# gashon/transformer-lm

Measured on AMD Instinct MI355X. Metric: BPE train input MB/s (32k vocab), train_bpe(path) end to end, higher is better.
Workload: dtype int64

## Files before the change

transformer-lm_amd/csrc/api.hip:

```cpp
#include <dlfcn.h>
#include <hip/hip_version.h>

#include <cerrno>
#include <cstdio>
#include <cstdlib>
#include <cstring>
#include <fstream>
#include <memory>
#include <mutex>
#include <string_view>
#include <unordered_map>
#include <unordered_set>
#include <string>
#include <vector>

#include "count.h"
#include "drive.h"
#include "internal.h"

namespace bpe {

namespace {
thread_local std::string g_err;
thread_local int g_errno = 0;
// ... 134 lines not shown
}

}

extern "C" {

int bpe_abi_version(void) { return BPE355_ABI_VERSION; }

int bpe_runtime_info(int* compiled_hip_version, int* runtime_hip_version, char* runtime_path, size_t cap) {
    if (compiled_hip_version) *compiled_hip_version = HIP_VERSION;
    int rv = 0;
    const hipError_t e = hipRuntimeGetVersion(&rv);
    if (runtime_hip_version) *runtime_hip_version = e == hipSuccess ? rv : 0;
    if (runtime_path && cap) {
        runtime_path[0] = '\0';
        Dl_info di{};
        if (dladdr(reinterpret_cast<void*>(&hipRuntimeGetVersion), &di) && di.dli_fname)
            std::snprintf(runtime_path, cap, "%s", di.dli_fname);
    }
    return e == hipSuccess ? BPE_OK : BPE_E_HIP;
}
const char* bpe_last_error(void) { return bpe::g_err.c_str(); }
int bpe_last_errno(void) { return bpe::g_errno; }
void bpe_set_timing(int enable) { bpe::g_timing = enable != 0; }

int bpe_release_device_memory(int device, size_t* freed_bytes) {
    return bpe::guarded([&] {
        if (freed_bytes) *freed_bytes = 0;
        int n = 0;
        if (hipGetDeviceCount(&n) != hipSuccess) n = 0;
        BPE_REQUIRE(device < n, BPE_E_ARG, "device " + std::to_string(device) + " is not visible");
        size_t b = bpe::corpus_release(device);
        b += bpe::scratch_release(device);
        if (freed_bytes) *freed_bytes = b;
    });
}

int bpe_device_count(void) {
    int n = 0;
    if (hipGetDeviceCount(&n) != hipSuccess) return 0;
    int k = 0;
    for (int i = 0; i < n; ++i) {
        hipDeviceProp_t p;
        if (hipGetDeviceProperties(&p, i) == hipSuccess && std::strncmp(p.gcnArchName, "gfx950", 6) == 0) ++k;
    }
    return k;
}

int bpe_train_device(const uint8_t* d_data, size_t n, int vocab_size, const char* const* specials,
                     int n_specials, bpe_comm* comm, void* hip_stream, bpe_result** out) {
    if (n && !d_data) return bpe::guarded([] { throw bpe::Error{BPE_E_ARG, "data is NULL"}; });
    return train_common(d_data, n, vocab_size, specials, n_specials, comm, hip_stream, out);
}

int bpe_train_buffer(const uint8_t* data, size_t n, int vocab_size, const char* const* specials,
                     int n_specials, bpe_comm* comm, bpe_result** out) {
    return bpe::guarded([&] {
        BPE_REQUIRE(out, BPE_E_ARG, "out is NULL");
        *out = nullptr;
        BPE_REQUIRE(!n || data, BPE_E_ARG, "data is NULL");
        bpe::DeviceGuard::require();
        auto sp = bpe::to_specials(specials, n_specials);
        const bpe::Source src = bpe::Source::memory(data, n);
        bpe::TrainOutput to;
        if (comm) bpe::train_source_comm(src, false, vocab_size, sp, comm->impl.get(), to);
        else bpe::train_source(src, vocab_size, sp, 1, to);
// ... 206 lines not shown
```

transformer-lm_amd/csrc/bpe_common.h:

```cpp
#pragma once

#include <hip/hip_runtime.h>

#include <cstddef>
#include <cstdint>
#include <string>

#include "../../include/bpe355.h"

namespace bpe {

void set_error(int code, const std::string& msg, int sys_errno = 0);
struct Error {
    int code;
    std::string msg;
    int sys_errno = 0;
};

#define BPE_HIP(expr)                                                                     \
    do {                                                                                  \
        hipError_t e_ = (expr);                                                           \
        if (e_ != hipSuccess)                                                             \
            throw ::bpe::Error{BPE_E_HIP, std::string(#expr) + ": " + hipGetErrorString(e_) + \
                                              " (" __FILE__ ":" + std::to_string(__LINE__) + ")"}; \
    } while (0)

#define BPE_REQUIRE(cond, code, msg)                          \
    do {                                                      \
        if (!(cond)) throw ::bpe::Error{(code), (msg)};       \
    } while (0)

template <class T>
struct DevBuf {
    T* p = nullptr;
    size_t n = 0;
    DevBuf() = default;
    explicit DevBuf(size_t count) { alloc(count); }
    DevBuf(const DevBuf&) = delete;
    DevBuf& operator=(const DevBuf&) = delete;
    DevBuf(DevBuf&& o) noexcept : p(o.p), n(o.n) { o.p = nullptr; o.n = 0; }
    DevBuf& operator=(DevBuf&& o) noexcept {
        if (this != &o) { release(); p = o.p; n = o.n; o.p = nullptr; o.n = 0; }
        return *this;
    }
    ~DevBuf() { release(); }
    void alloc(size_t count) {
        release();
        if (!count) return;
        const hipError_t e = hipMalloc(&p, count * sizeof(T));
        if (e == hipErrorOutOfMemory) {
            (void)hipGetLastError();
            p = nullptr;
            throw ::bpe::Error{BPE_E_NOMEM, "device allocation of " + std::to_string(count * sizeof(T)) +
                                                " bytes failed (out of memory)"};
        }
        BPE_HIP(e);
        n = count;
    }
    void reserve(size_t count) {
        if (count > n || !p) alloc(count);
    }
    void release() {
        if (p) (void)hipFree(p);
        p = nullptr;
        n = 0;
    }
    size_t bytes() const { return n * sizeof(T); }
};

enum : int { CLS_OTHER = 0, CLS_LETTER = 1, CLS_NUMBER = 2, CLS_SPACE = 3 };

__host__ __device__ inline uint64_t mix64(uint64_t z) {
    z ^= z >> 30; z *= 0xBF58476D1CE4E5B9ULL;
    z ^= z >> 27; z *= 0x94D049BB133111EBULL;
    return z ^ (z >> 31);
}

__device__ __forceinline__ unsigned wave_append(bool pred, unsigned* counter) {
    const unsigned long long m = __ballot(pred);
    if (!m) return ~0u;
    const int leader = __ffsll((long long)m) - 1;
    const unsigned lane = threadIdx.x & 63;
    unsigned base = 0;
    if ((int)lane == leader) base = atomicAdd(counter, (unsigned)__popcll(m));
    base = __shfl(base, leader);
    const unsigned below = __builtin_amdgcn_mbcnt_hi((unsigned)(m >> 32),
                                                     __builtin_amdgcn_mbcnt_lo((unsigned)m, 0u));
    return pred ? base + below : ~0u;
}

template <class T>
__device__ __forceinline__ T wave_sum(T v) {
    for (int o = 32; o > 0; o >>= 1) v += __shfl_xor(v, o);
    return v;
}

template <class T>
__device__ __forceinline__ T wave_max(T v) {
// ... 21 lines not shown
```

transformer-lm_amd/csrc/count.hip:

```cpp
#include <hip/hip_ext.h>

#include <algorithm>
#include <cstdlib>
#include <mutex>
#include <vector>

#include "count.h"
#include "pretok.h"
#include "prims.h"
#include "stage.h"
#include "stage2.h"
#include "tokstart.h"

#ifndef BPE355_COUNT_EARLY_PREFETCH
#define BPE355_COUNT_EARLY_PREFETCH 1
#endif

namespace bpe {

namespace {

constexpr int kCache2 = 512;
constexpr int kEpoch2 = 4;
constexpr unsigned kKeep2 = 2;
// ... 736 lines not shown
            } else {
                ++i;
            }
    }
    if (drop.empty()) return bytes;
    int cur = 0;
    BPE_HIP(hipGetDevice(&cur));
    for (auto& x : drop) {
        (void)hipSetDevice(x->dev);
        x.reset();
    }
    BPE_HIP(hipSetDevice(cur));
    return bytes;
}

void scratch_give(std::unique_ptr<Arrays3> x) {
    if (!x) return;
    std::lock_guard<std::mutex> g(scratch().m);
    scratch().free_.push_back(std::move(x));
}

RecPoolOwner::~RecPoolOwner() {
    scratch_give(std::move(rec));
    scratch_give(std::move(B));
}

void RecPoolOwner::init(size_t n_bytes, unsigned grid, hipStream_t s) {
    size_t want = std::max<size_t>(n_bytes / 10, (size_t)grid * kPageRecs);
    if (const char* e = std::getenv("BPE355_REC_POOL")) want = (size_t)std::atof(e);
    int dev = 0;
    BPE_HIP(hipGetDevice(&dev));
    size_t free_b = 0, total_b = 0;
    BPE_HIP(hipMemGetInfo(&free_b, &total_b));
    const size_t avail = free_b + scratch_cached_bytes(dev);
    const size_t reserve = std::max<size_t>(total_b / 16, n_bytes / 2);
    size_t fit = avail > reserve ? (avail - reserve) / (6 * sizeof(uint64_t) + 1) : 0;
    if (const char* e = std::getenv("BPE355_REC_POOL_FIT")) fit = (size_t)std::atof(e);
    if (fit < want) {
        if (fit < (size_t)grid * kPageRecs / 4)
            throw Error{BPE_E_NOMEM, "record pool: " + std::to_string(avail) + " bytes of device memory free"};
        want = fit;
    }
    max_pages = (unsigned)std::max<size_t>(1, std::min<size_t>((want + kPageRecs - 1) / kPageRecs, 1u << 30));
    const size_t cap = (size_t)max_pages * kPageRecs;
    if (std::getenv("BPE355_REC_POOL_FAIL"))
        throw Error{BPE_E_NOMEM, "record pool allocation failed (BPE355_REC_POOL_FAIL)"};
    rec = scratch_take(cap);
    page_used.alloc(max_pages);
    page_ch.alloc((size_t)max_pages * kCoarse);
    n_pages.alloc(1);
    wg_page.alloc(grid);
    wg_used.alloc(grid);
    wg_ch.alloc((size_t)grid * kCoarse);
    BPE_HIP(hipMemsetAsync(wg_ch.p, 0, 4ull * grid * kCoarse, s));
    held.alloc(max_pages);
    done.alloc(max_pages);
    lw_per_wg = (unsigned)std::min<size_t>(1u << 24, std::max<size_t>(1024, n_bytes / 1024 / grid + 1));
    if (const char* e = std::getenv("BPE355_LONG_SEG")) lw_per_wg = (unsigned)std::max(1, std::atoi(e));
    lw.alloc((size_t)lw_per_wg * grid);
    lw_n.alloc(grid);
    BPE_HIP(hipMemsetAsync(lw_n.p, 0, 4ull * grid, s));
    B = scratch_take(cap);
    if (B->d.n < cap) B->d.alloc(cap);
    max_tiles = max_pages + kCoarse;
    coff.alloc((size_t)kCoarse * max_pages);
    ctot.alloc(kCoarse);
    cbase.alloc(kCoarse + 1);
// ... 77 lines not shown
```

transformer-lm_amd/csrc/drive.hip:

```cpp
#include <fcntl.h>
#include <sys/stat.h>
#include <unistd.h>

#include <rccl/rccl.h>

#include <algorithm>
#include <atomic>
#include <condition_variable>
#include <cerrno>
#include <chrono>
#include <cstdio>
#include <cstring>
#include <exception>
#include <memory>
#include <mutex>
#include <thread>
#include <vector>

#include "drive.h"

namespace bpe {

namespace {

// ... 116 lines not shown
    corpus_cache().free_.push_back(std::move(x));
}

[[noreturn]] void io_error(int en, const std::string& what) {
    throw Error{BPE_E_IO, what + ": " + std::strerror(en), en};
}

}

size_t corpus_release(int dev) {
    std::vector<std::unique_ptr<CorpusBuf>> drop;
    size_t bytes = 0;
    {
        std::lock_guard<std::mutex> g(corpus_cache().m);
        auto& f = corpus_cache().free_;
        for (size_t i = 0; i < f.size();)
            if (dev < 0 || f[i]->dev == dev) {
                bytes += f[i]->b.bytes();
                drop.push_back(std::move(f[i]));
                f.erase(f.begin() + i);
            } else {
                ++i;
            }
    }
    if (drop.empty()) return bytes;
    int cur = 0;
    BPE_HIP(hipGetDevice(&cur));
    for (auto& x : drop) {
        (void)hipSetDevice(x->dev);
        x->b.release();
    }
    BPE_HIP(hipSetDevice(cur));
    return bytes;
}

int io_threads() {
    static const int t = [] {
        int n = 8;
        if (const char* e = std::getenv("BPE355_IO_THREADS")) n = std::atoi(e);
        return std::max(1, std::min(n, 16));
    }();
    return t;
}

static int dma_streams() {
    static const int t = [] {
        int n = 2;
        if (const char* e = std::getenv("BPE355_DMA_STREAMS")) n = std::atoi(e);
        return std::max(1, std::min(n, 16));
    }();
    return t;
}

namespace {
struct DmaStreams {
    std::vector<hipStream_t> s;
    DmaStreams(int device, int n, bool low_priority = false) {
        int cur = 0;
        BPE_HIP(hipGetDevice(&cur));
        BPE_HIP(hipSetDevice(device));
        s.resize(n, nullptr);
        int least = 0, greatest = 0;
        if (low_priority) BPE_HIP(hipDeviceGetStreamPriorityRange(&least, &greatest));
        hipError_t e = hipSuccess;
        for (auto& x : s)
            if (e == hipSuccess)
// ... 264 lines not shown
        cv.notify_all();
    }
    bool wait_prefix(size_t k) {
        std::unique_lock<std::mutex> lk(m);
        cv.wait(lk, [&] { return prefix >= k || failed; });
        return !failed;
    }
};

size_t segment_bytes() {
    const char* e = std::getenv("BPE355_SEG_MB");
    return (size_t)(e ? std::max(1, std::atoi(e)) : 256) << 20;
}

std::vector<size_t> segment_cuts(const Source& src, size_t off, size_t len, size_t seg) {
    std::vector<size_t> cut{0};
    std::vector<uint8_t> win(1u << 16);
    for (size_t want = seg; want + seg / 2 < len; want += seg) {
        const size_t lo = want - std::min(want, win.size() - 2);
        const size_t hi = want + 2;
        src.read(off + lo, hi - lo, win.data());
        const size_t p = bpe_safe_split(win.data(), hi - lo, want - lo);
        if (p > 0 && lo + p > cut.back()) cut.push_back(lo + p);
    }
    cut.push_back(len);
    return cut;
}

}

bool load_and_count(const Source& src, size_t off, size_t len, uint8_t* d_dst, int device, int threads,
                    hipStream_t stream, Prepared& pre) {
    const auto t0 = std::chrono::steady_clock::now();
    const std::vector<size_t> cut = segment_cuts(src, off, len, segment_bytes());
    const size_t chunks = (len + kStageChunk - 1) / kStageChunk;
    ChunkTrack track(chunks);
    const int t_n = (int)std::max<size_t>(1, std::min<size_t>((size_t)threads, chunks));
    std::atomic<size_t> next{0};
    std::vector<std::exception_ptr> errs(t_n);
    DmaStreams dma(device, dma_streams());
    auto reader = [&](int t) {
        const hipStream_t s = dma.pick(t);
        void* buf[2] = {nullptr, nullptr};
        size_t last[2] = {~(size_t)0, ~(size_t)0};
        try {
            BPE_HIP(hipSetDevice(device));
            for (int k = 0; k < 2; ++k) buf[k] = pool().get();
            for (int k = 0;; k ^= 1) {
                const size_t i = next.fetch_add(1);
                if (i >= chunks) break;
                if (last[k] != ~(size_t)0) BPE_HIP(hipEventSynchronize(track.ev[last[k]]));
                const size_t lo = i * kStageChunk, n = std::min(kStageChunk, len - lo);
                src.read(off + lo, n, static_cast<uint8_t*>(buf[k]));
                BPE_HIP(hipMemcpyAsync(d_dst + lo, buf[k], n, hipMemcpyHostToDevice, s));
                BPE_HIP(hipEventRecord(track.ev[i], s));
                last[k] = i;
                track.mark(i);
            }
        } catch (...) {
            errs[t] = std::current_exception();
            next.store(chunks);
            track.fail();
            (void)hipStreamSynchronize(s);
        }
        for (int k = 0; k < 2; ++k) {
            if (last[k] != ~(size_t)0) (void)hipEventSynchronize(track.ev[last[k]]);
// ... 194 lines not shown
```

transformer-lm_amd/csrc/train.hip:

```cpp
#include <hip/hip_ext.h>

#include <algorithm>
#include <chrono>
#include <climits>
#include <cstdio>
#include <cstdlib>
#include <cstring>
#include <set>
#include <unordered_map>

#include "internal.h"
#include "prims.h"

namespace bpe {

namespace {

constexpr unsigned kPresent = 1u, kInC = 2u;
enum : int { HALT_NONE = 0, HALT_REBUILD = 1, HALT_DONE = 2, HALT_HOST = 3 };
enum : unsigned { ERR_PAIRS_FULL = 1u, ERR_C_FULL = 2u, ERR_POOL = 4u };
constexpr unsigned long long kPolyP = 0x100000001B3ULL * 0x9E3779B97F4A7C15ULL | 1ULL;
constexpr int kNumCls = 4;
constexpr int kHistReplicas = 16;

struct RoundState {
    int halt;
    int round;
    int n_rounds;
    int ntok;
    long long T;
    unsigned nC, capC, c_limit, probe_merge_done;
    unsigned nC_base;
    int cur_round, cur_ntok;
    unsigned cur_a, cur_b, cur_new, cur_slot;
    long long cur_cnt;
    int new_is_new;
    unsigned err;
    unsigned n_single;
    unsigned n_single_new;
    unsigned pool_used, pool_cap;
    unsigned long long pair_used;
    unsigned long long scan_slots;
    int nparts;
    unsigned probe_apply_done;
    unsigned long long* probe;
    int host_round;
    unsigned single_limit;
    unsigned max_len;
    int max_batch;
    unsigned long long pair_limit;
    long long narrow_limit;
};

struct Partial {
    long long cnt;
    unsigned long long ka, kb;
// ... 2226 lines not shown
    __syncthreads();
    if (threadIdx.x == 0) {
        s_base = s_n ? atomicAdd(n_words, s_n) : 0u;
        if (s_ml) atomicMax(max_len, s_ml);
    }
    __syncthreads();
    unsigned idx = s_base + at;
#pragma unroll
    for (unsigned u = 0; u < kCollectPer; ++u) {
        if (!((keepm >> u) & 1u)) continue;
        const size_t s = s0 + (size_t)u * kCollectThreads;
        w_off[idx] = off[u]; w_len[idx] = len[u]; w_cnt[idx] = kv[2 * s + 1];
        ++idx;
    }
}

__global__ void k_len_u64(const uint32_t* __restrict__ w_len, unsigned n, unsigned long long* __restrict__ o) {
    const unsigned i = blockIdx.x * blockDim.x + threadIdx.x;
    if (i < n) o[i] = w_len[i];
}

template <class TokT>
__global__ void k_fill_words(const uint8_t* __restrict__ text, const unsigned long long* __restrict__ w_off,
                             const uint32_t* __restrict__ w_len, const unsigned long long* __restrict__ beg,
                             unsigned n, TokT* __restrict__ tok) {
    const unsigned w = blockIdx.x * blockDim.x + threadIdx.x;
    if (w >= n) return;
    const unsigned long long bg = beg[w];
    const uint32_t len = w_len[w];
    const uint8_t* src = text + w_off[w];
    for (uint32_t i = 0; i < len; ++i) tok[bg + i] = (TokT)src[i];
}

__global__ void k_hist_words(const unsigned long long* __restrict__ w_off, const uint32_t* __restrict__ w_len,
                             const unsigned long long* __restrict__ w_cnt, const uint8_t* __restrict__ text,
                             unsigned n, unsigned long long* __restrict__ hist) {
    const unsigned w = blockIdx.x * blockDim.x + threadIdx.x;
    if (w >= n) return;
    const uint8_t* src = text + w_off[w];
    const uint32_t len = w_len[w];
    const unsigned long long c = w_cnt[w];
    unsigned long long* h = hist + (size_t)(blockIdx.x % kHistReplicas) * 65536;
    unsigned prev = src[0];
    for (uint32_t i = 1; i < len; ++i) {
        const unsigned cur = src[i];
        atomicAdd(&h[prev * 256 + cur], c);
        prev = cur;
    }
}

__global__ void k_hist_reduce(unsigned long long* __restrict__ hist) {
    const unsigned i = blockIdx.x * blockDim.x + threadIdx.x;
    if (i >= 65536) return;
    unsigned long long s = 0;
    for (int r = 0; r < kHistReplicas; ++r) s += hist[(size_t)r * 65536 + i];
    hist[i] = s;
}

__global__ void k_init_pairs(const unsigned long long* __restrict__ hist, PairsDev P,
                             RoundState* st) {
    const unsigned i = blockIdx.x * blockDim.x + threadIdx.x;
    if (i >= 65536) return;
    const long long c = (long long)hist[i];
    if (c <= 0) return;
    bool ins;
    const size_t s = pair_slot(P, pair_key(i >> 8, i & 255u), st, &ins);
    if (s == ~(size_t)0) return;
    P.cnt[s] = c;
    P.flag[s] = kPresent;
}

__global__ void k_init_tokens(ToksDev K) {
    const unsigned i = threadIdx.x;
    K.pool[i] = (uint8_t)i;
    K.off[i] = i;
    K.len[i] = 1;
    K.hash[i] = i;
    K.pw[i] = kPolyP;
    K.key8[i] = (unsigned long long)i << 56;
    __syncthreads();
    if (i == 0) {
        for (unsigned t = 0; t < 256; ++t) {
            unsigned s = (unsigned)mix64(t) & K.map_mask;
            while (K.map[s] != 0) s = (s + 1) & K.map_mask;
            K.map[s] = map_entry(t, t);
        }
    }
}

template <class TokT>
__device__ __forceinline__ void word_at(const WordsDev<TokT>& W, unsigned g, int* c, unsigned* i) {
    unsigned acc = 0;
    for (int k = 0; k < kNumCls; ++k) {
        if (g < acc + W.c[k].n) { *c = k; *i = g - acc; return; }
        acc += W.c[k].n;
    }
    *c = kNumCls;
    *i = g - acc;
}

template <class TokT>
__device__ __forceinline__ uint32_t word_len(const WordsDev<TokT>& W, int c, unsigned i) {
    return c < kNumCls ? (uint32_t)W.c[c].slot[(size_t)i * slot_w(c)] : W.llen[i];
}

struct MoveCounts {
    unsigned n[kNumCls + 1];
    unsigned fill[kNumCls + 1];
    unsigned long long long_tokens, long_fill;
};

constexpr unsigned kMoveBlocks = 1024;
constexpr int kMoveK = kNumCls + 1;

__device__ __forceinline__ unsigned move_per_block(unsigned total) { return (total + kMoveBlocks - 1) / kMoveBlocks; }

template <class TokT>
__device__ __forceinline__ int move_class(const WordsDev<TokT>& W, unsigned g, unsigned total, int* c, unsigned* i,
                                          uint32_t* len) {
    int d = -1;
// ... 280 lines not shown
    const size_t i = (size_t)blockIdx.x * blockDim.x + threadIdx.x;
    if (i >= ocap) return;
    const unsigned long long k = okey[i];
    if (!k) return;
    bool ins;
    const size_t s = pair_slot(P, k, st, &ins);
    if (s == ~(size_t)0) return;
    P.cnt[s] = ocnt[i];
    P.flag[s] = oflag[i] & kPresent;
}

double ms_since(std::chrono::steady_clock::time_point t0) {
    return std::chrono::duration<double, std::milli>(std::chrono::steady_clock::now() - t0).count();
}

template <class TokT>
struct HostWords {
    DevBuf<TokT> slot[kNumCls];
    DevBuf<unsigned long long> cnt[kNumCls];
    unsigned n[kNumCls] = {0, 0, 0, 0};
    DevBuf<TokT> ltok;
    DevBuf<unsigned long long> lbeg, lcnt;
    DevBuf<uint32_t> llen;
    unsigned ln = 0;
    unsigned total() const { return n[0] + n[1] + n[2] + n[3] + ln; }
    WordsDev<TokT> dev() const {
        WordsDev<TokT> W{};
        for (int c = 0; c < kNumCls; ++c) W.c[c] = SlotCls<TokT>{slot[c].p, cnt[c].p, n[c], 0, 0, 0};
        W.ltok = ltok.p; W.lbeg = lbeg.p; W.llen = llen.p; W.lcnt = lcnt.p; W.ln = ln;
        return W;
    }
};

template <class TokT>
class MergeLoop {
   public:
    MergeLoop(hipStream_t stream, Comm* comm, const uint8_t* text, int n_rounds, TrainOutput& out)
        : s_(stream), comm_(comm), text_(text), n_rounds_(n_rounds), out_(out) {}
    ~MergeLoop() {
        if (snap_st_) (void)hipHostFree(snap_st_);
        if (snap_ti_) (void)hipHostFree(snap_ti_);
        for (auto e : blk_ev_)
            if (e) (void)hipEventDestroy(e);
    }
    MergeLoop(const MergeLoop&) = delete;
    MergeLoop& operator=(const MergeLoop&) = delete;

    void build_words(const WordCounts& wc, const std::vector<std::string>& specials);
    void run();

   private:
    static constexpr int kBatch = 64;
    static constexpr int kTrips = 32;
    int trips_ = 8;
    static_assert(2 * kTrips <= kBatch, "two blocks' timing events fit the event pool");
    static constexpr int kArgBlocks = 64;
    static constexpr unsigned kCScanBlocks = 64;
    unsigned nparts_ = 0;
    static constexpr int kTimingStride = 8;
    static constexpr unsigned long long kTarget = 4096;
    static constexpr size_t kPairLoadDiv = 2;

    void alloc_pairs(size_t cap);
    void grow_pairs();
    void ensure_pool(unsigned need);
    void push_state() { BPE_HIP(hipMemcpyAsync(st_.p, &hs_, sizeof(hs_), hipMemcpyHostToDevice, s_)); }
    void pull_state() {
        BPE_HIP(hipMemcpyAsync(&hs_, st_.p, sizeof(hs_), hipMemcpyDeviceToHost, s_));
        BPE_HIP(hipStreamSynchronize(s_));
    }
    int rebuild();
    void exhaustion();
    void compact();
    void layout_blocks();
    void build_index();
    PairsDev pairs() const { return PairsDev{pkey_.p, pcnt_.p, pflag_.p, pcap_ - 1, C_.p}; }
// ... 21 lines not shown
    unsigned trip_grid_ = 1;
    unsigned merge_grid_ = 1;
    unsigned merge_grid_cur_ = 0;
    double scan_bytes_ = 0, long_bytes_ = 0;
    unsigned long long long_tokens_ = 0;
    unsigned n_live_ = 0;
    DevBuf<unsigned long long> hist_;
    size_t pcap_ = 0;
    DevBuf<unsigned long long> pkey_;
    DevBuf<long long> pcnt_;
    DevBuf<unsigned> pflag_;
    DevBuf<uint4> C_;
    unsigned tok_cap_ = 0;
    size_t lr_member_ = 0;
    DevBuf<unsigned> tb_, tbc_;
    CellMarks cm_{};
    DevBuf<uint8_t> pool_;
    DevBuf<uint32_t> toff_, tlen_;
    DevBuf<unsigned long long> tmap_;
    DevBuf<unsigned long long> thash_, tpw_, tkey8_;
    DevBuf<unsigned long long> LR_;
    DevBuf<Partial> part_;
    DevBuf<uint32_t> m_a_, m_b_, m_new_, m_mode_;
    bool batched_ = false;
    bool fused_ = false;
    int max_batch_ = kMaxBatch;
    long long trips_launched_ = 0, trips_run_ = 0, rounds_batched_ = 0;
    std::unique_ptr<std::vector<int>> trip_log_;
    DevBuf<BatchState> bs_;
    DevBuf<Batch> batch_;
    DevBuf<unsigned long long> dbg_, sig_;
    DevBuf<uint32_t> tags_;
    DevBuf<int> trip_info_;
    RoundState* snap_st_ = nullptr;
    int* snap_ti_ = nullptr;
    RoundState* snap_st_dev_ = nullptr;
    int* snap_ti_dev_ = nullptr;
    hipEvent_t blk_ev_[2] = {nullptr, nullptr};
    long long slot_base_[2] = {0, 0};
    void launch_block(int slot, bool timing, std::vector<hipEvent_t>& ev);
    unsigned merge_grid() const;
    void finish_block(int slot, bool timing, std::vector<hipEvent_t>& ev, double& k1_ms, double& k1_bytes,
                      long long& k1_launches);
    DevBuf<unsigned long long> probe_;
    void report_probe();
    DevBuf<Partial> list_;
    static constexpr unsigned kApplyBatchBlocks = kApplyGrid;
    void reset_tags();

    DevBuf<long long> m_cnt_;
    DevBuf<RebuildStats> rs_;
    DevBuf<uint32_t> ilist_, ibeg_, ilen_;
    DevBuf<uint32_t> ix_cnt_, ix_pos_, ix_keys_, ix_vals_, ix_keys2_;
    DevBuf<uint8_t> ix_tmp_;
    HostWords<TokT> spare_;
    unsigned cls_cap_[kNumCls] = {};
    bool cls_cap_set_ = false;
    DevBuf<MoveCounts> move_counts_;
    DevBuf<unsigned> move_blk_;
    IndexDev idev_{};
    int next_index_round_ = 256;
};

template <class TokT>
void MergeLoop<TokT>::build_words(const WordCounts& wc, const std::vector<std::string>& specials) {
    std::string spb;
// ... 15 lines not shown
                       wc.pos.p, wc.cap, text_, d_spb.p, d_spo.p, d_spl.p, (int)specials.size(),
                       w_off.p, w_len.p, w_cnt.p, cnts.p, cnts.p + 1);
    BPE_HIP(hipGetLastError());
    unsigned h2[2];
    BPE_HIP(hipMemcpyAsync(h2, cnts.p, 8, hipMemcpyDeviceToHost, s_));
    BPE_HIP(hipStreamSynchronize(s_));
    n_words_ = h2[0];
    max_len_ = h2[1];
    const unsigned n = n_words_;
    hist_.alloc((size_t)kHistReplicas * 65536);
    BPE_HIP(hipMemsetAsync(hist_.p, 0, hist_.bytes(), s_));
    HostWords<TokT>& H = words_;
    unsigned long long total_tok = 0;
    H.ln = n;
    H.llen.alloc(std::max(n, 1u));
    H.lbeg.alloc(std::max(n, 1u));
    H.lcnt.alloc(std::max(n, 1u));
    if (n) {
        DevBuf<unsigned long long> len64(n);
        hipLaunchKernelGGL(k_len_u64, dim3(ceil_div(n, 256)), dim3(256), 0, s_, w_len.p, n, len64.p);
        exclusive_sum(len64.p, H.lbeg.p, n, s_);
        unsigned long long last[2];
        BPE_HIP(hipMemcpyAsync(&last[0], H.lbeg.p + n - 1, 8, hipMemcpyDeviceToHost, s_));
        BPE_HIP(hipMemcpyAsync(&last[1], len64.p + n - 1, 8, hipMemcpyDeviceToHost, s_));
        BPE_HIP(hipStreamSynchronize(s_));
        total_tok = last[0] + last[1];
    }
    H.ltok.alloc(std::max<unsigned long long>(total_tok, 1));
    if (n) {
        BPE_HIP(hipMemcpyAsync(H.llen.p, w_len.p, n * 4ull, hipMemcpyDeviceToDevice, s_));
        BPE_HIP(hipMemcpyAsync(H.lcnt.p, w_cnt.p, n * 8ull, hipMemcpyDeviceToDevice, s_));
        hipLaunchKernelGGL(k_fill_words<TokT>, dim3(ceil_div(n, 256)), dim3(256), 0, s_, text_, w_off.p,
                           w_len.p, H.lbeg.p, n, H.ltok.p);
        hipLaunchKernelGGL(k_hist_words, dim3(ceil_div(n, 256)), dim3(256), 0, s_, w_off.p,
                           w_len.p, w_cnt.p, text_, n, hist_.p);
        BPE_HIP(hipGetLastError());
    }
    hipLaunchKernelGGL(k_hist_reduce, dim3(256), dim3(256), 0, s_, hist_.p);
    out_.stats.n_words = n;
    out_.stats.n_word_tokens = (int64_t)total_tok;
    BPE_HIP(hipStreamSynchronize(s_));
    n_live_ = n;
    compact();
}

template <class TokT>
void MergeLoop<TokT>::compact() {
    HostWords<TokT>& H = words_;
    const unsigned total = H.total();
    DevBuf<MoveCounts>& mc = move_counts_;
    DevBuf<unsigned>& blk = move_blk_;
    mc.reserve(1);
    blk.reserve((size_t)kMoveBlocks * kMoveK);
    BPE_HIP(hipMemsetAsync(mc.p, 0, sizeof(MoveCounts), s_));
    const WordsDev<TokT> src = H.dev();
    if (total) {
        hipLaunchKernelGGL(k_move_count<TokT>, dim3(kMoveBlocks), dim3(256), 0, s_, src, total, blk.p, mc.p);
        hipLaunchKernelGGL(k_move_scan, dim3(1), dim3(kMoveBlocks), 0, s_, blk.p, mc.p);
    }
    MoveCounts h{};
    BPE_HIP(hipMemcpyAsync(&h, mc.p, sizeof(h), hipMemcpyDeviceToHost, s_));
    BPE_HIP(hipStreamSynchronize(s_));
    HostWords<TokT> D = std::move(spare_);
    if (!cls_cap_set_) {
        unsigned ge = h.n[kNumCls];
        for (int c = kNumCls - 1; c >= 0; --c) cls_cap_[c] = ge += h.n[c];
        cls_cap_set_ = true;
    }
// ... 243 lines not shown
        batched_ = !sharded() && max_batch_ >= 1;
    }
    lr_member_ = (2ull * tok_cap_ + 63) / 64 * 64;
    LR_.alloc(2 * (batched_ ? (size_t)kMaxBatch : 1) * lr_member_);
    BPE_HIP(hipMemsetAsync(LR_.p, 0, LR_.bytes(), s_));
    if (batched_) {
        const unsigned dense_tok = [] {
            const char* e = std::getenv("BPE355_DENSE_TOK");
            const unsigned v = e ? (unsigned)std::max(0, std::atoi(e)) : 2048u;
            return std::max(128u, v / 32 * 32);
        }();
        const unsigned tbw = ceil_div(tok_cap_, 1024u);
        const bool marks = tbw <= kTBMax && !(std::getenv("BPE355_CELL_MARKS") && std::getenv("BPE355_CELL_MARKS")[0] == '0');
        const unsigned sparse_from = [&] {
            const char* e = std::getenv("BPE355_SPARSE_FROM");
            return std::max(dense_tok, e ? (unsigned)std::max(0, std::atoi(e)) : 16384u);
        }();
        cm_ = CellMarks{nullptr, nullptr, marks ? tbw : 0u, dense_tok, sparse_from, nullptr};
        if (marks) {
            tb_.alloc(2ull * kTBRep * kMaxBatch * tbw);
            tbc_.alloc((size_t)kMaxBatch * tbw);
            BPE_HIP(hipMemsetAsync(tb_.p, 0, tb_.bytes(), s_));
            BPE_HIP(hipMemsetAsync(tbc_.p, 0, tbc_.bytes(), s_));
            cm_.tb = tb_.p;
            cm_.tbc = tbc_.p;
        }
    }
    if (batched_) {
        bs_.alloc(1);
        BPE_HIP(hipMemsetAsync(bs_.p, 0, sizeof(BatchState), s_));
        batch_.alloc(1);
        BPE_HIP(hipMemsetAsync(batch_.p, 0, sizeof(Batch), s_));
        trip_info_.alloc(2 * kTI * kTrips);
        if (!snap_st_) {
            BPE_HIP(hipHostMalloc(reinterpret_cast<void**>(&snap_st_), 2 * sizeof(RoundState), hipHostMallocCoherent));
            BPE_HIP(hipHostMalloc(reinterpret_cast<void**>(&snap_ti_), 2 * kTI * kTrips * sizeof(int),
                                  hipHostMallocCoherent));
            BPE_HIP(hipHostGetDevicePointer(reinterpret_cast<void**>(&snap_st_dev_), snap_st_, 0));
            BPE_HIP(hipHostGetDevicePointer(reinterpret_cast<void**>(&snap_ti_dev_), snap_ti_, 0));
            for (auto& e : blk_ev_) BPE_HIP(hipEventCreateWithFlags(&e, hipEventDisableTiming));
        }
        if (const char* e = std::getenv("BPE355_TRIPS")) trips_ = std::max(1, std::min(std::atoi(e), kTrips));
        list_.alloc(2 * kListCap);
        const char* fe = std::getenv("BPE355_FOLD");
        fused_ = fe && fe[0] == '1';
    }
    if (batched_ && std::getenv("BPE355_CHECK_MARKS")) {
        dbg_.alloc(8);
        BPE_HIP(hipMemsetAsync(dbg_.p, 0, dbg_.bytes(), s_));
        sig_.alloc(1 + kApplyBatchBlocks);
        BPE_HIP(hipMemsetAsync(sig_.p, 0, sig_.bytes(), s_));
        cm_.sig = sig_.p;
    }
    const char* trip_log_path = std::getenv("BPE355_TRIP_LOG");
    if (batched_ && trip_log_path) trip_log_.reset(new std::vector<int>());
    m_a_.alloc(n_rounds_); m_b_.alloc(n_rounds_); m_new_.alloc(n_rounds_); m_mode_.alloc(n_rounds_);
    const char* round_log = std::getenv("BPE355_ROUND_LOG");
    if (round_log) m_cnt_.alloc(n_rounds_);
    toff_.alloc(tok_cap_); tlen_.alloc(tok_cap_);
    thash_.alloc(tok_cap_); tpw_.alloc(tok_cap_); tkey8_.alloc(tok_cap_);
    tmap_.alloc(next_pow2(16ull * tok_cap_));
    BPE_HIP(hipMemsetAsync(tmap_.p, 0, tmap_.bytes(), s_));
    const unsigned pool_cap = std::max(1u << 16, 64u * std::max(max_len_, 8u));
    pool_.alloc(pool_cap);

    if (sharded()) {
        comm_->allreduce_i64(reinterpret_cast<int64_t*>(hist_.p), 65536, s_);
        std::vector<int64_t> ml(comm_->nranks, 0);
        ml[comm_->rank] = max_len_;
        DevBuf<int64_t> d_ml(ml.size());
        BPE_HIP(hipMemcpyAsync(d_ml.p, ml.data(), ml.size() * 8, hipMemcpyHostToDevice, s_));
        comm_->allreduce_i64(d_ml.p, ml.size(), s_);
        BPE_HIP(hipMemcpyAsync(ml.data(), d_ml.p, ml.size() * 8, hipMemcpyDeviceToHost, s_));
// ... 536 lines not shown
        v[3 * comm->rank] = mine->code;
        v[3 * comm->rank + 1] = mine->sys_errno;
        const size_t p = mine->msg.find("position ");
        v[3 * comm->rank + 2] = p == std::string::npos ? 0 : std::stoll(mine->msg.substr(p + 9));
    }
    DevBuf<int64_t> d(v.size());
    BPE_HIP(hipMemcpyAsync(d.p, v.data(), v.size() * 8, hipMemcpyHostToDevice, stream));
    comm->allreduce_i64(d.p, v.size(), stream);
    BPE_HIP(hipMemcpyAsync(v.data(), d.p, v.size() * 8, hipMemcpyDeviceToHost, stream));
    BPE_HIP(hipStreamSynchronize(stream));
    for (int r = 0; r < R; ++r) {
        const int code = (int)v[3 * r];
        if (!code) continue;
        if (r == comm->rank && mine) throw *mine;
        if (code == BPE_E_UTF8)
            throw Error{code, "'utf-8' codec can't decode byte at position " + std::to_string(v[3 * r + 2])};
        throw Error{code, "rank " + std::to_string(r) + " failed before training (code " + std::to_string(code) + ")",
                    (int)v[3 * r + 1]};
    }
}

}

bool per_round_exchange() {
    const char* ex = std::getenv("BPE355_EXCHANGE");
    return ex && std::string(ex) == "rounds";
}

void train_on_device(const uint8_t* d_raw, size_t n, int vocab_size,
                     const std::vector<std::string>& specials, Comm* comm, hipStream_t stream,
                     TrainOutput& out, const TrainOpts& opt, Prepared* pre) {
    const auto t0 = std::chrono::steady_clock::now();
    out = TrainOutput{};
    DevBuf<uint8_t> scratch;
    size_t tn = 0;
    const uint8_t* text = nullptr;
    const bool several = comm && comm->nranks > 1;
    WordCounts wc;
    float count_ms = 0;
    std::chrono::steady_clock::time_point t1;
    {
        Error err{0, ""};
        bool failed = opt.has_pending;
        if (failed) err = opt.pending;
        if (!failed && pre) {
            text = pre->text;
            tn = pre->n;
            wc = std::move(pre->wc);
            count_ms = pre->count_kernel_ms;
            out.stats.t_prepare_ms = pre->t_prepare_ms;
            out.stats.n_bytes = (int64_t)tn;
            t1 = std::chrono::steady_clock::now() - std::chrono::duration_cast<std::chrono::steady_clock::duration>(
                                                         std::chrono::duration<double, std::milli>(pre->t_count_ms));
        } else if (!failed) {
            try {
                text = prepare_text(d_raw, n, scratch, &tn, stream);
                out.stats.t_prepare_ms = ms_since(t0);
                out.stats.n_bytes = (int64_t)tn;
                t1 = std::chrono::steady_clock::now();
                count_words(text, tn, wc, stream, timing_enabled() ? &count_ms : nullptr);
            } catch (const Error& e) {
                if (!several && !opt.slab_offset) throw;
                err = e;
                failed = true;
            }
        }
// ... 62 lines not shown
```

Baseline: 25450.

## Cache device blocks and pinned snapshots across calls; LDS-privatize pair histogram

Routes DevBuf allocations through a per-device block cache: frees made inside a BlockScope are deferred and later recycled, so repeated hipMalloc/hipFree calls in load_and_count and train_on_device can be skipped across invocations. Pinned host snapshot buffers and events are pooled in the same way. The byte-pair histogram kernel becomes grid-strided with a shared-memory 96x96 bin for printable bytes, which reduces global atomics, and the initial map fill is parallelized with CAS. The cost is extra memory held between calls and a stream synchronize when each scope exits.

```diff
diff --git a/transformer-lm_amd/csrc/api.hip b/transformer-lm_amd/csrc/api.hip
--- a/transformer-lm_amd/csrc/api.hip
+++ b/transformer-lm_amd/csrc/api.hip
@@ -190,6 +190,7 @@
         BPE_REQUIRE(device < n, BPE_E_ARG, "device " + std::to_string(device) + " is not visible");
         size_t b = bpe::corpus_release(device);
         b += bpe::scratch_release(device);
+        b += bpe::block_release(device);
         if (freed_bytes) *freed_bytes = b;
     });
 }
diff --git a/transformer-lm_amd/csrc/bpe_common.h b/transformer-lm_amd/csrc/bpe_common.h
--- a/transformer-lm_amd/csrc/bpe_common.h
+++ b/transformer-lm_amd/csrc/bpe_common.h
@@ -30,40 +30,47 @@
         if (!(cond)) throw ::bpe::Error{(code), (msg)};       \
     } while (0)
 
+void* block_alloc(size_t bytes, size_t* cap_bytes);
+void block_free(void* p, size_t cap_bytes) noexcept;
+size_t block_cached_bytes(int dev);
+size_t block_release(int dev);
+struct BlockScope {
+    explicit BlockScope(hipStream_t stream);
+    ~BlockScope();
+    BlockScope(const BlockScope&) = delete;
+    BlockScope& operator=(const BlockScope&) = delete;
+    hipStream_t s;
+};
+
 template <class T>
 struct DevBuf {
     T* p = nullptr;
     size_t n = 0;
+    size_t cap_b = 0;
     DevBuf() = default;
     explicit DevBuf(size_t count) { alloc(count); }
     DevBuf(const DevBuf&) = delete;
     DevBuf& operator=(const DevBuf&) = delete;
-    DevBuf(DevBuf&& o) noexcept : p(o.p), n(o.n) { o.p = nullptr; o.n = 0; }
+    DevBuf(DevBuf&& o) noexcept : p(o.p), n(o.n), cap_b(o.cap_b) { o.p = nullptr; o.n = 0; o.cap_b = 0; }
     DevBuf& operator=(DevBuf&& o) noexcept {
-        if (this != &o) { release(); p = o.p; n = o.n; o.p = nullptr; o.n = 0; }
+        if (this != &o) { release(); p = o.p; n = o.n; cap_b = o.cap_b; o.p = nullptr; o.n = 0; o.cap_b = 0; }
         return *this;
     }
     ~DevBuf() { release(); }
     void alloc(size_t count) {
         release();
         if (!count) return;
-        const hipError_t e = hipMalloc(&p, count * sizeof(T));
-        if (e == hipErrorOutOfMemory) {
-            (void)hipGetLastError();
-            p = nullptr;
-            throw ::bpe::Error{BPE_E_NOMEM, "device allocation of " + std::to_string(count * sizeof(T)) +
-                                                " bytes failed (out of memory)"};
-        }
-        BPE_HIP(e);
+        p = static_cast<T*>(block_alloc(count * sizeof(T), &cap_b));
         n = count;
     }
     void reserve(size_t count) {
         if (count > n || !p) alloc(count);
     }
     void release() {
-        if (p) (void)hipFree(p);
+        if (p) block_free(p, cap_b);
         p = nullptr;
         n = 0;
+        cap_b = 0;
     }
     size_t bytes() const { return n * sizeof(T); }
 };
diff --git a/transformer-lm_amd/csrc/count.hip b/transformer-lm_amd/csrc/count.hip
--- a/transformer-lm_amd/csrc/count.hip
+++ b/transformer-lm_amd/csrc/count.hip
@@ -792,7 +792,7 @@
     BPE_HIP(hipGetDevice(&dev));
     size_t free_b = 0, total_b = 0;
     BPE_HIP(hipMemGetInfo(&free_b, &total_b));
-    const size_t avail = free_b + scratch_cached_bytes(dev);
+    const size_t avail = free_b + scratch_cached_bytes(dev) + block_cached_bytes(dev);
     const size_t reserve = std::max<size_t>(total_b / 16, n_bytes / 2);
     size_t fit = avail > reserve ? (avail - reserve) / (6 * sizeof(uint64_t) + 1) : 0;
     if (const char* e = std::getenv("BPE355_REC_POOL_FIT")) fit = (size_t)std::atof(e);
diff --git a/transformer-lm_amd/csrc/drive.hip b/transformer-lm_amd/csrc/drive.hip
--- a/transformer-lm_amd/csrc/drive.hip
+++ b/transformer-lm_amd/csrc/drive.hip
@@ -172,6 +172,147 @@
     }
     BPE_HIP(hipSetDevice(cur));
     return bytes;
+}
+
+namespace {
+struct Block {
+    void* p;
+    size_t cap;
+    int dev;
+};
+struct BlockCache {
+    std::mutex m;
+    std::vector<Block> free_;
+};
+BlockCache& block_cache() {
+    static BlockCache* c = new BlockCache;
+    return *c;
+}
+void free_blocks(std::vector<Block>& v) {
+    if (v.empty()) return;
+    int cur = 0;
+    (void)hipGetDevice(&cur);
+    for (auto& b : v) {
+        (void)hipSetDevice(b.dev);
+        (void)hipFree(b.p);
+    }
+    (void)hipSetDevice(cur);
+    v.clear();
+}
+struct BlockThread {
+    int depth = 0;
+    std::vector<Block> pending;
+    ~BlockThread() { free_blocks(pending); }
+};
+BlockThread& block_thread() {
+    thread_local BlockThread t;
+    return t;
+}
+}
+
+void* block_alloc(size_t bytes, size_t* cap_bytes) {
+    BlockThread& t = block_thread();
+    int dev = 0;
+    BPE_HIP(hipGetDevice(&dev));
+    if (t.depth > 0) {
+        BlockCache& c = block_cache();
+        std::lock_guard<std::mutex> g(c.m);
+        size_t best = c.free_.size();
+        for (size_t i = 0; i < c.free_.size(); ++i) {
+            const Block& b = c.free_[i];
+            if (b.dev == dev && b.cap >= bytes && b.cap / 2 <= bytes && (best == c.free_.size() || b.cap < c.free_[best].cap))
+                best = i;
+        }
+        if (best < c.free_.size()) {
+            const Block b = c.free_[best];
+            c.free_[best] = c.free_.back();
+            c.free_.pop_back();
+            *cap_bytes = b.cap;
+            return b.p;
+        }
+    }
+    void* p = nullptr;
+    hipError_t e = hipMalloc(&p, bytes);
+    if (e == hipErrorOutOfMemory) {
+        (void)hipGetLastError();
+        block_release(dev);
+        std::vector<Block> mine;
+        for (size_t i = 0; i < t.pending.size();)
+            if (t.pending[i].dev == dev) {
+                mine.push_back(t.pending[i]);
+                t.pending[i] = t.pending.back();
+                t.pending.pop_back();
+            } else {
+                ++i;
+            }
+        free_blocks(mine);
+        p = nullptr;
+        e = hipMalloc(&p, bytes);
+    }
+    if (e == hipErrorOutOfMemory) {
+        (void)hipGetLastError();
+        throw Error{BPE_E_NOMEM, "device allocation of " + std::to_string(bytes) + " bytes failed (out of memory)"};
+    }
+    BPE_HIP(e);
+    *cap_bytes = bytes;
+    return p;
+}
+
+void block_free(void* p, size_t cap_bytes) noexcept {
+    BlockThread& t = block_thread();
+    int dev = 0;
+    if (t.depth > 0 && hipGetDevice(&dev) == hipSuccess) {
+        try {
+            t.pending.push_back(Block{p, cap_bytes, dev});
+            return;
+        } catch (...) {
+        }
+    }
+    (void)hipFree(p);
+}
+
+size_t block_cached_bytes(int dev) {
+    BlockCache& c = block_cache();
+    std::lock_guard<std::mutex> g(c.m);
+    size_t b = 0;
+    for (auto& x : c.free_)
+        if (x.dev == dev) b += x.cap;
+    return b;
+}
+
+size_t block_release(int dev) {
+    std::vector<Block> drop;
+    size_t bytes = 0;
+    {
+        BlockCache& c = block_cache();
+        std::lock_guard<std::mutex> g(c.m);
+        for (size_t i = 0; i < c.free_.size();)
+            if (dev < 0 || c.free_[i].dev == dev) {
+                bytes += c.free_[i].cap;
+                drop.push_back(c.free_[i]);
+                c.free_[i] = c.free_.back();
+                c.free_.pop_back();
+            } else {
+                ++i;
+            }
+    }
+    free_blocks(drop);
+    return bytes;
+}
+
+BlockScope::BlockScope(hipStream_t stream) : s(stream) { ++block_thread().depth; }
+
+BlockScope::~BlockScope() {
+    BlockThread& t = block_thread();
+    if (--t.depth > 0 || t.pending.empty()) return;
+    if (hipStreamSynchronize(s) != hipSuccess) {
+        free_blocks(t.pending);
+        return;
+    }
+    BlockCache& c = block_cache();
+    std::lock_guard<std::mutex> g(c.m);
+    c.free_.insert(c.free_.end(), t.pending.begin(), t.pending.end());
+    t.pending.clear();
 }
 
 int io_threads() {
@@ -502,6 +643,7 @@
 bool load_and_count(const Source& src, size_t off, size_t len, uint8_t* d_dst, int device, int threads,
                     hipStream_t stream, Prepared& pre) {
     const auto t0 = std::chrono::steady_clock::now();
+    BlockScope blocks(stream);
     const std::vector<size_t> cut = segment_cuts(src, off, len, segment_bytes());
     const size_t chunks = (len + kStageChunk - 1) / kStageChunk;
     ChunkTrack track(chunks);
diff --git a/transformer-lm_amd/csrc/train.hip b/transformer-lm_amd/csrc/train.hip
--- a/transformer-lm_amd/csrc/train.hip
+++ b/transformer-lm_amd/csrc/train.hip
@@ -6,6 +6,8 @@
 #include <cstdio>
 #include <cstdlib>
 #include <cstring>
+#include <memory>
+#include <mutex>
 #include <set>
 #include <unordered_map>
 
@@ -22,6 +24,7 @@
 constexpr unsigned long long kPolyP = 0x100000001B3ULL * 0x9E3779B97F4A7C15ULL | 1ULL;
 constexpr int kNumCls = 4;
 constexpr int kHistReplicas = 16;
+constexpr unsigned kHistLo = 0x20, kHistSide = 96, kHistThreads = 1024, kHistPerCu = 2;
 
 struct RoundState {
     int halt;
@@ -2314,21 +2317,46 @@
     for (uint32_t i = 0; i < len; ++i) tok[bg + i] = (TokT)src[i];
 }
 
-__global__ void k_hist_words(const unsigned long long* __restrict__ w_off, const uint32_t* __restrict__ w_len,
-                             const unsigned long long* __restrict__ w_cnt, const uint8_t* __restrict__ text,
-                             unsigned n, unsigned long long* __restrict__ hist) {
-    const unsigned w = blockIdx.x * blockDim.x + threadIdx.x;
-    if (w >= n) return;
-    const uint8_t* src = text + w_off[w];
-    const uint32_t len = w_len[w];
-    const unsigned long long c = w_cnt[w];
+__global__ void __launch_bounds__(kHistThreads)
+k_hist_words(const unsigned long long* __restrict__ w_off, const uint32_t* __restrict__ w_len,
+             const unsigned long long* __restrict__ w_cnt, const uint8_t* __restrict__ text,
+             unsigned n, unsigned long long* __restrict__ hist) {
+    __shared__ unsigned long long s_bin[kHistSide * kHistSide];
+    for (unsigned i = threadIdx.x; i < kHistSide * kHistSide; i += kHistThreads) s_bin[i] = 0;
+    __syncthreads();
     unsigned long long* h = hist + (size_t)(blockIdx.x % kHistReplicas) * 65536;
-    unsigned prev = src[0];
-    for (uint32_t i = 1; i < len; ++i) {
-        const unsigned cur = src[i];
-        atomicAdd(&h[prev * 256 + cur], c);
-        prev = cur;
-    }
+    for (size_t w = (size_t)blockIdx.x * kHistThreads + threadIdx.x; w < n; w += (size_t)gridDim.x * kHistThreads) {
+        const uint8_t* src = text + w_off[w];
+        const uint32_t len = w_len[w];
+        const unsigned long long c = w_cnt[w];
+        unsigned prev = src[0];
+        for (uint32_t i = 1; i < len; i += 8) {
+            unsigned b[8];
+#pragma unroll
+            for (uint32_t u = 0; u < 8; ++u) b[u] = i + u < len ? src[i + u] : 0u;
+#pragma unroll
+            for (uint32_t u = 0; u < 8; ++u) {
+                if (i + u >= len) break;
+                const unsigned cur = b[u];
+                const unsigned p = prev - kHistLo, q = cur - kHistLo;
+                if (p < kHistSide && q < kHistSide) atomicAdd(&s_bin[p * kHistSide + q], c);
+                else atomicAdd(&h[prev * 256 + cur], c);
+                prev = cur;
+            }
+        }
+    }
+    __syncthreads();
+    for (unsigned i = threadIdx.x; i < kHistSide * kHistSide; i += kHistThreads) {
+        const unsigned long long v = s_bin[i];
+        if (v) atomicAdd(&h[(i / kHistSide + kHistLo) * 256 + i % kHistSide + kHistLo], v);
+    }
+}
+
+static unsigned hist_grid() {
+    int dev = 0, n_cu = 0;
+    BPE_HIP(hipGetDevice(&dev));
+    BPE_HIP(hipDeviceGetAttribute(&n_cu, hipDeviceAttributeMultiprocessorCount, dev));
+    return kHistPerCu * (unsigned)std::max(1, n_cu);
 }
 
 __global__ void k_hist_reduce(unsigned long long* __restrict__ hist) {
@@ -2360,14 +2388,8 @@
     K.hash[i] = i;
     K.pw[i] = kPolyP;
     K.key8[i] = (unsigned long long)i << 56;
-    __syncthreads();
-    if (i == 0) {
-        for (unsigned t = 0; t < 256; ++t) {
-            unsigned s = (unsigned)mix64(t) & K.map_mask;
-            while (K.map[s] != 0) s = (s + 1) & K.map_mask;
-            K.map[s] = map_entry(t, t);
-        }
-    }
+    unsigned s = (unsigned)mix64(i) & K.map_mask;
+    while (atomicCAS(&K.map[s], 0ull, map_entry(i, i)) != 0ull) s = (s + 1) & K.map_mask;
 }
 
 template <class TokT>
@@ -2714,16 +2736,70 @@
     }
 };
 
+struct SnapSet {
+    int dev = 0;
+    void* st = nullptr;
+    void* ti = nullptr;
+    void* st_dev = nullptr;
+    void* ti_dev = nullptr;
+    hipEvent_t ev[2] = {nullptr, nullptr};
+};
+struct SnapCache {
+    std::mutex m;
+    std::vector<SnapSet*> free_;
+};
+SnapCache& snap_cache() {
+    static SnapCache* c = new SnapCache;
+    return *c;
+}
+SnapSet* snap_take(size_t st_bytes, size_t ti_bytes) {
+    int dev = 0;
+    BPE_HIP(hipGetDevice(&dev));
+    {
+        std::lock_guard<std::mutex> g(snap_cache().m);
+        auto& f = snap_cache().free_;
+        for (size_t i = 0; i < f.size(); ++i)
+            if (f[i]->dev == dev) {
+                SnapSet* x = f[i];
+                f.erase(f.begin() + i);
+                return x;
+            }
+    }
+    std::unique_ptr<SnapSet> x(new SnapSet);
+    x->dev = dev;
+    auto drop = [&] {
+        if (x->st) (void)hipHostFree(x->st);
+        if (x->ti) (void)hipHostFree(x->ti);
+        for (auto e : x->ev)
+            if (e) (void)hipEventDestroy(e);
+    };
+    try {
+        BPE_HIP(hipHostMalloc(&x->st, st_bytes, hipHostMallocCoherent));
+        BPE_HIP(hipHostMalloc(&x->ti, ti_bytes, hipHostMallocCoherent));
+        BPE_HIP(hipHostGetDevicePointer(&x->st_dev, x->st, 0));
+        BPE_HIP(hipHostGetDevicePointer(&x->ti_dev, x->ti, 0));
+        for (auto& e : x->ev) BPE_HIP(hipEventCreateWithFlags(&e, hipEventDisableTiming));
+    } catch (...) {
+        drop();
+        throw;
+    }
+    return x.release();
+}
+void snap_give(SnapSet* x) {
+    if (!x) return;
+    std::lock_guard<std::mutex> g(snap_cache().m);
+    snap_cache().free_.push_back(x);
+}
+
 template <class TokT>
 class MergeLoop {
    public:
     MergeLoop(hipStream_t stream, Comm* comm, const uint8_t* text, int n_rounds, TrainOutput& out)
         : s_(stream), comm_(comm), text_(text), n_rounds_(n_rounds), out_(out) {}
     ~MergeLoop() {
-        if (snap_st_) (void)hipHostFree(snap_st_);
-        if (snap_ti_) (void)hipHostFree(snap_ti_);
-        for (auto e : blk_ev_)
-            if (e) (void)hipEventDestroy(e);
+        if (!snap_) return;
+        (void)hipStreamSynchronize(s_);
+        snap_give(snap_);
     }
     MergeLoop(const MergeLoop&) = delete;
     MergeLoop& operator=(const MergeLoop&) = delete;
@@ -2811,6 +2887,7 @@
     DevBuf<unsigned long long> dbg_, sig_;
     DevBuf<uint32_t> tags_;
     DevBuf<int> trip_info_;
+    SnapSet* snap_ = nullptr;
     RoundState* snap_st_ = nullptr;
     int* snap_ti_ = nullptr;
     RoundState* snap_st_dev_ = nullptr;
@@ -2892,8 +2969,8 @@
         BPE_HIP(hipMemcpyAsync(H.lcnt.p, w_cnt.p, n * 8ull, hipMemcpyDeviceToDevice, s_));
         hipLaunchKernelGGL(k_fill_words<TokT>, dim3(ceil_div(n, 256)), dim3(256), 0, s_, text_, w_off.p,
                            w_len.p, H.lbeg.p, n, H.ltok.p);
-        hipLaunchKernelGGL(k_hist_words, dim3(ceil_div(n, 256)), dim3(256), 0, s_, w_off.p,
-                           w_len.p, w_cnt.p, text_, n, hist_.p);
+        hipLaunchKernelGGL(k_hist_words, dim3(std::min(ceil_div(n, kHistThreads), hist_grid())),
+                           dim3(kHistThreads), 0, s_, w_off.p, w_len.p, w_cnt.p, text_, n, hist_.p);
         BPE_HIP(hipGetLastError());
     }
     hipLaunchKernelGGL(k_hist_reduce, dim3(256), dim3(256), 0, s_, hist_.p);
@@ -3203,13 +3280,14 @@
         batch_.alloc(1);
         BPE_HIP(hipMemsetAsync(batch_.p, 0, sizeof(Batch), s_));
         trip_info_.alloc(2 * kTI * kTrips);
-        if (!snap_st_) {
-            BPE_HIP(hipHostMalloc(reinterpret_cast<void**>(&snap_st_), 2 * sizeof(RoundState), hipHostMallocCoherent));
-            BPE_HIP(hipHostMalloc(reinterpret_cast<void**>(&snap_ti_), 2 * kTI * kTrips * sizeof(int),
-                                  hipHostMallocCoherent));
-            BPE_HIP(hipHostGetDevicePointer(reinterpret_cast<void**>(&snap_st_dev_), snap_st_, 0));
-            BPE_HIP(hipHostGetDevicePointer(reinterpret_cast<void**>(&snap_ti_dev_), snap_ti_, 0));
-            for (auto& e : blk_ev_) BPE_HIP(hipEventCreateWithFlags(&e, hipEventDisableTiming));
+        if (!snap_) {
+            snap_ = snap_take(2 * sizeof(RoundState), 2 * kTI * kTrips * sizeof(int));
+            snap_st_ = static_cast<RoundState*>(snap_->st);
+            snap_ti_ = static_cast<int*>(snap_->ti);
+            snap_st_dev_ = static_cast<RoundState*>(snap_->st_dev);
+            snap_ti_dev_ = static_cast<int*>(snap_->ti_dev);
+            blk_ev_[0] = snap_->ev[0];
+            blk_ev_[1] = snap_->ev[1];
         }
         if (const char* e = std::getenv("BPE355_TRIPS")) trips_ = std::max(1, std::min(std::atoi(e), kTrips));
         list_.alloc(2 * kListCap);
@@ -3812,6 +3890,7 @@
                      TrainOutput& out, const TrainOpts& opt, Prepared* pre) {
     const auto t0 = std::chrono::steady_clock::now();
     out = TrainOutput{};
+    BlockScope blocks(stream);
     DevBuf<uint8_t> scratch;
     size_t tn = 0;
     const uint8_t* text = nullptr;
```

Measured after the change: 26560 (median of 6 runs). +4.4%, better.
